# ktonal/mimikit

Measured on AMD Instinct MI355X. Metric: audio samples/sec generated (WaveNet 256-ch mu-law, 16kHz), higher is better.
Workload: dtype f32; 1 GPU; wavenet_cfg4: WaveNet blocks=(10, 10, 10) x 256 ch, 1 cond input(s), mu-law-256, 16 kHz; clips_per_gpu=32, global_clips=32, prompt_samples=3072, decode=greedy, parallelism=clip-shard x1

## Files before the change

### mimikit_amd/csrc/gemm.hip

```cpp
#include "mmk_common.h"
#include "plan_util.h"

namespace mmk {

typedef float f32x4 __attribute__((ext_vector_type(4)));
typedef const __attribute__((address_space(1))) f32x4* gf32x4_ptr;

constexpr int kGemmThreads = 512;
constexpr int kGemmBM = 64, kGemmBN = 128;

__global__ __launch_bounds__(kGemmThreads) void gemm_f32_kernel(const float* __restrict__ A, int64_t lda, int64_t a_batch,
                                                                const float* __restrict__ Wp, float* __restrict__ C,
                                                                int64_t ldc, int64_t c_batch, int M, int n_tiles, int N,
                                                                int K, int k_chunks) {
  extern __shared__ __attribute__((aligned(16))) char smem_raw[];
  float* as = reinterpret_cast<float*>(smem_raw);
  const int ldk = k_chunks * 16 + 4;
  const int tid = threadIdx.x, lane = tid & 63;
  const int wave = __builtin_amdgcn_readfirstlane(tid >> 6);
  const int m_first = blockIdx.y * kGemmBM;
  const int tile = blockIdx.x * (kGemmBN / 16) + wave;
  A += (int64_t)blockIdx.z * a_batch;
  C += (int64_t)blockIdx.z * c_batch;
  const int k4 = k_chunks * 4;
// ... 47 lines not shown
      for (int i = 0; i < 4; ++i) if (col0 + c + i < N) dst[i] = v[i];
  }
}

int launch_gemm_f32(const float* A, int64_t lda, int64_t a_batch, const float* Wp, int n_tiles, int k_chunks, int N, int K,
                    float* C, int64_t ldc, int64_t c_batch, int M, int batch, hipStream_t stream) {
  if (M <= 0 || batch <= 0 || n_tiles <= 0) return MMK_OK;
  size_t lds = (size_t)kGemmBM * (k_chunks * 16 + 4) * sizeof(float);
  const size_t lds_out = (size_t)kGemmBM * (kGemmBN + 4) * sizeof(float);
  if (lds < lds_out) lds = lds_out;
  if (lds > 160 * 1024) return fail(MMK_ERR_UNSUPPORTED, "gemm: K=%d does not fit the LDS stage", K);
  if ((lda % 4) != 0 || (reinterpret_cast<uintptr_t>(A) & 15) != 0) return fail(MMK_ERR_UNSUPPORTED, "gemm: A must be 16-byte aligned with lda %% 4 == 0");
  dim3 grid((n_tiles + kGemmBN / 16 - 1) / (kGemmBN / 16), (M + kGemmBM - 1) / kGemmBM, batch), block(kGemmThreads);
  hipLaunchKernelGGL(gemm_f32_kernel, grid, block, lds, stream, A, lda, a_batch, Wp, C, ldc, c_batch, M, n_tiles, N, K, k_chunks);
  MMK_HIP(hipGetLastError());
  return MMK_OK;
}

constexpr int kTgThreads = 256;
constexpr int kTgBM = 64, kTgBN = 64;
constexpr int kTgCh = 4;
constexpr int kTgLd = kTgCh * 16 + 4;

template <bool WLDS>
__global__ __launch_bounds__(kTgThreads, 2) void gemm_bias_act_kernel(const float* __restrict__ A, int64_t lda, const float* __restrict__ Wp,
                                                                 const float* __restrict__ bias, float* __restrict__ C, int64_t ldc,
                                                                 int M, int n_tiles, int N, int K, int k_chunks, int act, GemmRowMap rm,
                                                                 int k_split, float* __restrict__ partial) {
  extern __shared__ __attribute__((aligned(16))) char smem_raw[];
  float* as = reinterpret_cast<float*>(smem_raw);

  const int tid = threadIdx.x, lane = tid & 63;
  const int wave = __builtin_amdgcn_readfirstlane(tid >> 6);
  const int wm = wave >> 1, wn = wave & 1;
  const int m_first = blockIdx.y * kTgBM;
  const int tile0 = blockIdx.x * (kTgBN / 16) + wn * 2;
  const int a_row = 16 * wave + (lane >> 4) + 4 * ((lane >> 2) & 3), a_col = (lane & 3) * 4;
  const int r0 = m_first + a_row;
  const float* a0 = A + (int64_t)(r0 < M ? r0 : M - 1) * lda + a_col;
  f32x4 va[kTgCh];
  auto load_a = [&](int stage) {
#pragma unroll
    for (int cc = 0; cc < kTgCh; ++cc) {
      const int c = stage * kTgCh + cc;
      const int k = c * 16 + a_col;
      if (k + 3 < K) {
        va[cc] = *reinterpret_cast<const f32x4*>(a0 + c * 16);
      } else {
        for (int i = 0; i < 4; ++i) va[cc][i] = k + i < K ? a0[c * 16 + i] : 0.f;
      }
    }
  };
  auto store_a = [&](int buf) {
    float* dst = as + buf * (kTgBM * kTgLd);
#pragma unroll
    for (int cc = 0; cc < kTgCh; ++cc) {
      *reinterpret_cast<f32x4*>(dst + a_row * kTgLd + cc * 16 + a_col) = va[cc];
    }
  };
  const int t0 = tile0 < n_tiles ? tile0 : n_tiles - 1, t1 = tile0 + 1 < n_tiles ? tile0 + 1 : n_tiles - 1;
  gf32x4_ptr w0 = (gf32x4_ptr)(uintptr_t)Wp + (int64_t)t0 * k_chunks * 64 + lane;
  gf32x4_ptr w1 = (gf32x4_ptr)(uintptr_t)Wp + (int64_t)t1 * k_chunks * 64 + lane;
  f32x4 wc[WLDS ? 1 : kTgCh][2], wx[WLDS ? 1 : kTgCh][2];
  auto load_w = [&](int stage, f32x4 (&w)[WLDS ? 1 : kTgCh][2]) {
    if constexpr (!WLDS) {
#pragma unroll
      for (int cc = 0; cc < kTgCh; ++cc) {
        const int c = stage * kTgCh + cc;
        const int cl = c < k_chunks ? c : k_chunks - 1;
        w[cc][0] = w0[(int64_t)cl * 64];
        w[cc][1] = w1[(int64_t)cl * 64];
      }
    }
  };
  f32x4* ws = reinterpret_cast<f32x4*>(as + 2 * kTgBM * kTgLd);
  const int tl = wn * 2 + wm;
  const int tg = blockIdx.x * (kTgBN / 16) + tl;
// ... 114 lines not shown
  if (rm.group > 0 && i >= rm.kept) return;
  float* dst = rm.group > 0 ? C + (int64_t)g * rm.group_stride + (int64_t)i * rm.row_stride : C + (int64_t)m * ldc;
  for (int col = threadIdx.x; col < N; col += blockDim.x) {
    float v = partial[(int64_t)m * np + col];
    for (int z = 1; z < k_split; ++z) v += partial[((int64_t)z * M + m) * np + col];
    dst[col] = apply_act(v + (bias ? bias[col] : 0.f), act);
  }
}

bool gemm_bias_act_supported(const float* A, int64_t lda, int M, int K) {
  static const int min_m = [] { const char* e = diag_only("MMK_GEMM_MIN_M"); return e ? atoi(e) : 128; }();
  return M >= min_m && K >= 16 && (lda % 4) == 0 && (reinterpret_cast<uintptr_t>(A) & 15) == 0;
}

int gemm_bias_act_k_split(int M, int n_tiles, int k_chunks, int forced = 0) {
  const int wgs = ((n_tiles + kTgBN / 16 - 1) / (kTgBN / 16)) * ((M + kTgBM - 1) / kTgBM);
  const int stages = (k_chunks + kTgCh - 1) / kTgCh;
  int ks = 1;
  while (ks * 2 <= stages && wgs * ks * 2 <= 512 && ks < 8) ks *= 2;
  if (forced > 0) ks = forced < stages ? forced : stages;
  return ks;
}

int64_t gemm_bias_act_partial_floats(int M, int n_tiles, int k_chunks) {
  const int ks = gemm_bias_act_k_split(M, n_tiles, k_chunks);
  return ks > 1 ? (int64_t)ks * M * n_tiles * 16 : 0;
}

int launch_gemm_bias_act(const float* A, int64_t lda, const float* Wp, const float* bias, int n_tiles, int k_chunks, int N, int K, float* C,
                         int64_t ldc, int M, int act, hipStream_t stream, GemmRowMap rm, float* partial, int64_t partial_floats, int forced_k_split) {
  if (M <= 0 || n_tiles <= 0) return MMK_OK;
  if (!gemm_bias_act_supported(A, lda, M, K)) return fail(MMK_ERR_UNSUPPORTED, "gemm_bias_act: needs M >= 128 and a 16-byte aligned A");
  int ks = partial ? gemm_bias_act_k_split(M, n_tiles, k_chunks, forced_k_split) : 1;
  if (ks > 1 && (int64_t)ks * M * n_tiles * 16 > partial_floats) ks = 1;
  dim3 grid((n_tiles + kTgBN / 16 - 1) / (kTgBN / 16), (M + kTgBM - 1) / kTgBM, ks), block(kTgThreads);
  const size_t lds = (size_t)2 * kTgBM * kTgLd * sizeof(float);
  const char* we = diag_only("MMK_GEMM_WLDS");
  if (!(we && we[0] == '0'))
    hipLaunchKernelGGL(gemm_bias_act_kernel<true>, grid, block, lds + (size_t)2 * 4 * kTgCh * 64 * 16, stream, A, lda, Wp, bias, C, ldc, M, n_tiles, N, K,
                       k_chunks, act, rm, ks, partial);
  else
    hipLaunchKernelGGL(gemm_bias_act_kernel<false>, grid, block, lds, stream, A, lda, Wp, bias, C, ldc, M, n_tiles, N, K, k_chunks, act, rm, ks, partial);
  MMK_HIP(hipGetLastError());
  if (ks > 1) {
    hipLaunchKernelGGL(gemm_split_reduce_kernel, dim3(M), dim3(256), 0, stream, partial, ks, M, n_tiles * 16, N, bias, C, ldc, act, rm);
    MMK_HIP(hipGetLastError());
  }
  return MMK_OK;
}

}

extern "C" int mmk_gemm_f32(const float* a, int64_t lda, int64_t a_batch, const float* packed_w, int32_t n_rows, int32_t k_cols, float* c,
                            int64_t ldc, int64_t c_batch, int32_t m_rows, int32_t batch, mmk_stream_t stream) {
  using namespace mmk;
  if (!a || !packed_w || !c || m_rows <= 0 || n_rows <= 0 || k_cols <= 0 || batch <= 0 || lda < k_cols || ldc < n_rows || a_batch < 0 ||
      c_batch < 0)
    return fail(MMK_ERR_INVALID, "gemm: bad arguments");
  if (batch > 1 && (a_batch % 4) != 0) return fail(MMK_ERR_UNSUPPORTED, "gemm: a_batch %% 4 != 0");
  return launch_gemm_f32(a, lda, a_batch, packed_w, (n_rows + 15) / 16, (k_cols + 15) / 16, n_rows, k_cols, c, ldc, c_batch, m_rows, batch,
                         (hipStream_t)stream);
}

extern "C" int64_t mmk_gemm_partial_floats(int32_t m_rows, int32_t n_rows, int32_t k_cols, int32_t k_split) {
  if (m_rows <= 0 || n_rows <= 0 || k_cols <= 0 || k_split < 0) return 0;
// ... 29 lines not shown
```

### mimikit_amd/csrc/mmk_common.h

```cpp
#pragma once
#include <hip/hip_runtime.h>
#include <stdint.h>
#include <stdio.h>
#include <string>
#include <vector>

#include "../../include/mmk.h"

namespace mmk {

void set_error(const char* fmt, ...);
int fail(int code, const char* fmt, ...);

#define MMK_HIP(call)                                                                         \
  do {                                                                                        \
    hipError_t e__ = (call);                                                                  \
    if (e__ != hipSuccess)                                                                    \
      return ::mmk::fail(MMK_ERR_HIP, "%s failed: %s (%s:%d)", #call, hipGetErrorString(e__), \
                         __FILE__, __LINE__);                                                 \
  } while (0)

#define MMK_TRY(expr)            \
  do {                           \
    int rc__ = (expr);           \
// ... 171 lines not shown
};
int launch_sample(const SampleArgs& a, hipStream_t stream);

int launch_stft1024(const float* x, int64_t x_row_stride, int batch, int64_t n_samples, int hop, int center, int reflect, int out_mode,
                    float* out, float* tprev, float momentum, hipStream_t stream);
int launch_stft2048(const float* x, int64_t x_row_stride, int batch, int64_t n_samples, int hop, int center, int reflect, int out_mode,
                    float* out, hipStream_t stream);
int launch_istft2048(const float* spec, const float* mag, int mode, int batch, int64_t n_frames, int hop, float* out, hipStream_t stream);
int launch_gla2048_iter(const float* wave_in, const float* mag, const float* tprev_in, float* tprev_out, float momentum, int batch,
                        int64_t n_frames, int hop, float* wave_out, hipStream_t stream);
int launch_stft_generic(const float* x, int64_t x_row_stride, int batch, int64_t n_samples, int n_fft, int hop, int center, int reflect,
                        int out_mode, float* out, float* tprev, float momentum, hipStream_t stream);
int launch_gemm_f32(const float* A, int64_t lda, int64_t a_batch, const float* Wp, int n_tiles, int k_chunks, int N, int K,
                    float* C, int64_t ldc, int64_t c_batch, int M, int batch, hipStream_t stream);
bool gemm_bias_act_supported(const float* A, int64_t lda, int M, int K);
struct GemmRowMap {
  int32_t group = 0, kept = 0;
  int64_t group_stride = 0, row_stride = 0;
};
int64_t gemm_bias_act_partial_floats(int M, int n_tiles, int k_chunks);
int launch_gemm_bias_act(const float* A, int64_t lda, const float* Wp, const float* bias, int n_tiles, int k_chunks, int N, int K, float* C,
                         int64_t ldc, int M, int act, hipStream_t stream, GemmRowMap rm = GemmRowMap(), float* partial = nullptr,
                         int64_t partial_floats = 0, int forced_k_split = 0);

bool skinny_linear_supported(const float* A, int64_t lda, int M, int K, int k_chunks);
int launch_skinny_linear(const float* A, int64_t lda, const float* Wp, const float* bias, int n_tiles, int k_chunks, int N, int K, float* C,
                         int64_t ldc, int M, int act, hipStream_t stream);

int launch_gru_cell(const float* gi, const float* gh, float* h, int M, int H, hipStream_t stream);
int launch_lstm_cell(const float* gates, int64_t gates_ld, const float* gadd, int64_t gadd_ld, float* h, int64_t h_ld,
                     float* c, int64_t c_ld, float* y, int64_t y_ld, int M, int H, hipStream_t stream);
int launch_rnn_tanh_cell(const float* g, float* h, int M, int H, hipStream_t stream);

}
```

### mimikit_amd/csrc/wavenet_plan.hip

```cpp
#include <stdlib.h>

#include "plan_util.h"
#include "wavenet_chain.h"
#include "wavenet_lpipe.h"
#include "wavenet_persist.h"
#include "wavenet_prefill.h"
#include "wavenet_spipe.h"
#include "wavenet_bpipe.h"

using namespace mmk;

constexpr int kBpipeMinClips = 105;
constexpr int kBpipeAlwaysClips = kSpMaxClips + 1;
static bool bpipe_by_default(int B) { return B >= kBpipeAlwaysClips || (B >= kBpipeMinClips && B % 2 != 0); }

struct WnCall {
  int M = 0;
  const void* in0 = nullptr;
  int64_t in0_rs = 0;
  const float* cond[MMK_MAX_COND] = {nullptr, nullptr, nullptr, nullptr};
  int64_t cond_rs[MMK_MAX_COND] = {0, 0, 0, 0};
  const float* temperature = nullptr;
  const float* uniforms = nullptr;
  int64_t uni_ld = 0;
// ... 23 lines not shown
  std::vector<float*> hist;
  std::vector<float*> cbuf;
  float* ybuf = nullptr;
  float* skipbuf = nullptr;
  float* hid[2] = {nullptr, nullptr};
  int64_t* tau = nullptr;

  hipStream_t cap_stream = nullptr;
  GraphCache gc;

  bool persistent = false;
  int Gc = 0, Gn = 0, Mg = 0, C1 = 0, n_logits_pad = 0;
  static constexpr int kCondBlock = 1024;
  std::vector<int64_t> ring_offset;
  std::vector<int> ring_mask;
  int64_t ring_floats_per_wg = 0;
  PackedLinear cond_all;
  WnLayerTab* layer_tab = nullptr;
  unsigned long long *gran_h = nullptr, *gran_y = nullptr, *gran_skip = nullptr, *gran_hid = nullptr,
                     *gran_logit = nullptr, *gran_idx = nullptr;
  int64_t gran_words = 0;
  float* h_rings = nullptr;
  float* cproj = nullptr;
  float* cpad = nullptr;
  int64_t cpad_rows = 0;
  float* condall = nullptr;
  float* zero_pad = nullptr;
  int64_t pf_P = 0;
  float *pf_h[2] = {nullptr, nullptr}, *pf_y = nullptr, *pf_c = nullptr;
  int32_t* err_flag = nullptr;
  unsigned* xcd_count = nullptr;
  bool xcd_local = false;
  bool chain = false;
  bool lpipe = false;
  unsigned long long *lp_xg = nullptr, *lp_cg = nullptr;
  int64_t lp_gran_words = 0;
  std::vector<PackedLinear> Ac;
  WnChainIter* iter_tab = nullptr;
  float* compose_scratch = nullptr;
  bool spipe = false;
  int last_pair = 0;
  bool bpipe = false;
  float *bp_img = nullptr, *bp_cst = nullptr;
  unsigned* bp_msg = nullptr;
  float *sp_img_chain = nullptr, *sp_img_helper = nullptr, *sp_cst_chain = nullptr, *sp_cst_helper = nullptr, *sp_head_w0 = nullptr, *sp_head_b0 = nullptr;
  unsigned *sp_msg = nullptr, *sp_hidmsg = nullptr, *sp_hidgrp = nullptr;
  WnSpRaw* sp_raw = nullptr;
  const float *sp_fc2_w = nullptr, *sp_fc2_b = nullptr;
// ... 39 lines not shown
      sp_head_b0 = c.take<float>(kSpH1);
      sp_f0p = c.take<float>((int64_t)kSpH1 * C);
      sp_fb0p = c.take<float>(kSpH1);
      sp_fc2p = c.take<float>((int64_t)(kSpQ + 1) * kSpH1);
      sp_fc2bp = c.take<float>(kSpLogitsLd);
      sp_logits = c.take<float>((int64_t)Bmax * kSpLogitsLd);
      if (n_cond == 2) {
        sp_w1cat = c.take<float>((int64_t)L * 2 * C * C1);
        sp_b1cat = c.take<float>((int64_t)L * 2 * C);
      }
      if (bpipe) {
        bp_img = c.take<float>(wn_bpipe_img_floats(L));
        bp_cst = c.take<float>(wn_bpipe_cst_floats(L));
        bp_msg = c.take<unsigned>(wn_bpipe_msg_words(L, Bmax));
      } else {
        sp_msg = c.take<unsigned>(wn_spipe_msg_words(L, C, Bmax) + wn_spipe_hidmsg_words(L, Bmax) + wn_spipe_hidgrp_words(Bmax));
        sp_hidmsg = sp_msg + (sp_msg ? wn_spipe_msg_words(L, C, Bmax) : 0);
        sp_hidgrp = sp_hidmsg + (sp_msg ? wn_spipe_hidmsg_words(L, Bmax) : 0);
      }
      sp_raw = c.take<WnSpRaw>(L);
    }
    h_rings = spipe ? nullptr : c.take<float>((int64_t)Gc * Gn * ring_floats_per_wg);
    cproj = C1 > 0 ? c.take<float>((int64_t)Bmax * kCondBlock * C1) : nullptr;
    if (C1 > 0) {
      int kmax = 16;
      for (int j = 0; j < n_cond; ++j) kmax = (int)round_up(cfg.cond_in_dim[j], 16) > kmax ? (int)round_up(cfg.cond_in_dim[j], 16) : kmax;
      const int64_t prompt_rows = round_up(rf, 32);
      cpad_rows = (int64_t)Bmax * (prompt_rows > kCondBlock ? prompt_rows : kCondBlock);
      cpad = c.take<float>(cpad_rows * kmax);
    }
    condall = (C1 > 0 && !spipe) ? c.take<float>((int64_t)Bmax * kCondBlock * L * 2 * C) : nullptr;
    if (C1 > 0 && !spipe) cond_all.carve(c, false);
    if (chain) {
      for (auto& pl : Ac) pl.carve(c, true);
      iter_tab = c.take<WnChainIter>(L + 1);
      compose_scratch = c.take<float>((int64_t)2 * C * C + 2 * C);
    }
    zero_pad = c.take<float>(64);
    pf_P = round_up(rf, 32);
    pf_h[0] = c.take<float>((int64_t)Bmax * pf_P * C);
    pf_h[1] = c.take<float>((int64_t)Bmax * pf_P * C);
    pf_y = c.take<float>((int64_t)Bmax * pf_P * C);
    pf_c = C1 > 0 ? c.take<float>((int64_t)Bmax * pf_P * C1) : nullptr;
  }

  void layout(Carver& c) {
    const bool bias = cfg.bias != 0;
    if (cfg.q_levels == 0) in0_lin.carve(c, true);
    for (auto& p : cond_lin) p.carve(c, true);
    for (auto& p : A) p.carve(c, bias);
    for (auto& p : Aff) p.carve(c, bias);
    affbuf = Aff.empty() ? nullptr : c.take<float>((int64_t)Bmax * 3 * C);
    for (auto& p : Bm)
// ... 687 lines not shown
      s.uniform_ld = call.uni_ld; s.uni_off = call.uni_off;
      if (k == 0) { s.out = (int64_t*)call.in0; s.out_row_stride = call.in0_rs; }
      else { s.out = reinterpret_cast<int64_t*>(const_cast<float*>(call.cond[k - 1])); s.out_row_stride = call.cond_rs[k - 1]; }
      s.out_tau_off = 1;
      s.tau_ptr = p->tau; s.tau_off = tau_off;
      MMK_TRY(launch_sample(s, st));
    }
  } else {
    LinearArgs a = {};
    p->out_lin.fill(a);
    a.seg[0].x = addr_static(x);
    a.seg[0].ld = p->head_in;
    a.M = M; a.tau_ptr = p->tau; a.tau_off = tau_off;
    a.epilogue = EPI_STORE; a.act = c.head_kind == 1 ? ACT_ABS : ACT_NONE;
    a.out = addr_time(call.in0, c.in_dim, 1, 1, 0);
    a.out_ld = call.in0_rs;
    MMK_TRY(launch_linear(a, st));
  }
  return MMK_OK;
}

static constexpr int kGraphSteps = 8;

__global__ void cond_compact_kernel(const float* __restrict__ src, int64_t clip_stride, int64_t t0, int K, int Kp, int n, int B, float* __restrict__ dst) {
  const int64_t e = (int64_t)blockIdx.x * blockDim.x + threadIdx.x;
  if (e >= (int64_t)B * n * Kp) return;
  const int k = (int)(e % Kp);
  const int64_t row = e / Kp;
  const int b = (int)(row / n), i = (int)(row - (int64_t)b * n);
  dst[e] = k < K ? src[(int64_t)b * clip_stride + (t0 + i) * K + k] : 0.f;
}

static int project_cond(mmk_wavenet_plan* p, const WnCall& call, int j, int col, int64_t t0, int64_t n, float* out, int64_t out_clip_stride, hipStream_t st) {
  const mmk_wavenet_config& c = p->cfg;
  const int K = c.cond_in_dim[j], Kp = (int)round_up(K, 16), B = call.M;
  const char* genv = p->tune.get("MMK_WN_COND_GEMM");
  const int64_t M = (int64_t)B * n;
  if (!(genv && genv[0] == '0') && p->cpad && M <= p->cpad_rows && M < ((int64_t)1 << 31) && gemm_bias_act_supported(p->cpad, Kp, (int)M, K)) {
    const int64_t total = M * Kp;
    hipLaunchKernelGGL(cond_compact_kernel, dim3((unsigned)((total + 255) / 256)), dim3(256), 0, st, call.cond[j], call.cond_rs[j], t0, K, Kp, (int)n, B, p->cpad);
    MMK_HIP(hipGetLastError());
    GemmRowMap rm;
    rm.group = (int)n; rm.kept = (int)n; rm.group_stride = out_clip_stride * p->C1; rm.row_stride = p->C1;
    return launch_gemm_bias_act(p->cpad, Kp, p->cond_lin[j].Wp, p->cond_lin[j].bias, p->cond_lin[j].n_tiles, p->cond_lin[j].k_chunks, c.cond_dim[j], K,
                                out + col, p->C1, (int)M, ACT_NONE, st, rm);
  }
  LinearArgs a = {};
  p->cond_lin[j].fill(a);
  a.seg[0].x = addr_static(call.cond[j] + t0 * K);
  a.seg[0].ld = K;
  a.M = (int)M; a.tau_ptr = nullptr; a.tau_off = 0;
  a.epilogue = EPI_STORE; a.act = ACT_NONE;
  a.out = addr_static(out + col);
  a.out_ld = p->C1;
  a.row_group = (int)n; a.x_group_stride = call.cond_rs[j]; a.out_group_stride = out_clip_stride * p->C1;
  return launch_linear(a, st);
}

static int run_persistent(mmk_wavenet_plan* p, const WnCall& call, int64_t tau0, int64_t n, bool with_head, hipStream_t st) {
  const mmk_wavenet_config& c = p->cfg;
  const MlpHead& h0 = p->heads[0];
  for (int64_t done = 0; done < n;) {
    const int64_t block = (p->lpipe && p->C1 == 0) ? ((int64_t)1 << 20) : (int64_t)p->kCondBlock;
    const int64_t nb = (n - done) < block ? (n - done) : block;
    const int64_t tau_b = tau0 + done;
    if (p->C1 > 0) {
      g_prof_tag = 2;
      for (int j = 0, col = 0; j < p->n_cond; col += c.cond_dim[j], ++j)
// ... 131 lines not shown
    a.h_rings = p->h_rings; a.err_flag = p->err_flag;
    {
      const char* senv = diag_only("MMK_WN_STAMPS");
      a.stamps = (senv && senv[0] == '1') ? reinterpret_cast<unsigned long long*>(p->tau + 8) : nullptr;
    }
    MMK_TRY(launch_wavenet_persist(a, st));
    done += nb;
  }
  return MMK_OK;
}

static int prefill(mmk_wavenet_plan* p, const WnCall& call, int64_t t_begin, int64_t t_end, hipStream_t st) {
  const mmk_wavenet_config& c = p->cfg;
  const int C = p->C, L = p->L, C1 = p->C1, B = call.M;
  const int64_t n = t_end - t_begin, P = p->pf_P;
  MMK_TRY(launch_wn_prefill_embed((const int64_t*)call.in0, call.in0_rs, t_begin, p->emb, c.q_levels, C, (int)n, p->pf_h[0],
                                  P * C, B, st));
  if (C1 > 0) {
    for (int j = 0, col = 0; j < p->n_cond; col += c.cond_dim[j], ++j)
      MMK_TRY(project_cond(p, call, j, col, t_begin, n, p->pf_c, P, st));
  }
  std::vector<int64_t> sfx(L, 0);
  for (int l = L - 2; l >= 0; --l) sfx[l] = sfx[l + 1] + p->dil[l + 1];
  int cur = 0;
  for (int l = 0; l < L; ++l) {
    const int d = p->dil[l];
    const int64_t t_lo = t_end - d > t_begin ? t_end - d : t_begin;
    if (p->lpipe || p->spipe)
      MMK_TRY(launch_wn_lpipe_scatter(p->pf_h[cur], P * C, t_begin, t_lo, (int)(t_end - t_lo), C, B, p->Bmax, p->hist[l], p->ring[l], st));
    else
      MMK_TRY(launch_wn_prefill_scatter(p->pf_h[cur], P * C, t_begin, t_lo, (int)(t_end - t_lo), C, B, p->Mg, p->Gc, p->Gn, p->h_rings,
                                        p->ring_floats_per_wg, p->ring_offset[l], p->ring_mask[l], st));
    if (l == L - 1) break;
    int64_t r_lo = t_end - sfx[l];
    if (r_lo < t_begin + d) r_lo = t_begin + d;
    if (r_lo >= t_end) break;
    const int64_t p0 = r_lo - t_begin;
    const int M = (int)(t_end - r_lo);
    const float* h = p->pf_h[cur];
    {
      WnPrefillArgs a = {};
      a.M = M; a.N = 2 * C; a.n_tiles = p->A[l].n_tiles; a.k_chunks = p->A[l].k_chunks;
      a.nseg = C1 > 0 ? 3 : 2;
      a.seg_k[0] = C; a.seg[0] = h + (p0 - d) * C; a.seg_ld[0] = C; a.seg_batch[0] = P * C;
      a.seg_k[1] = C; a.seg[1] = h + p0 * C; a.seg_ld[1] = C; a.seg_batch[1] = P * C;
      if (C1 > 0) { a.seg_k[2] = C1; a.seg[2] = p->pf_c + p0 * C1; a.seg_ld[2] = C1; a.seg_batch[2] = P * C1; }
      a.wp = p->A[l].Wp; a.bias = p->A[l].bias;
      a.out = p->pf_y + p0 * C; a.out_ld = C; a.out_batch = P * C;
      MMK_TRY(launch_wn_prefill(a, 0, B, st));
    }
    {
      WnPrefillArgs a = {};
      a.M = M; a.N = C; a.n_tiles = C / 16; a.k_chunks = p->Bm[l].k_chunks;
      a.nseg = 1;
      a.seg_k[0] = C; a.seg[0] = p->pf_y + p0 * C; a.seg_ld[0] = C; a.seg_batch[0] = P * C;
      a.wp = p->Bm[l].Wp; a.bias = p->Bm[l].bias;
      a.res_in = h + p0 * C; a.res_ld = C; a.res_batch = P * C;
      a.out = p->pf_h[cur ^ 1] + p0 * C; a.out_ld = C; a.out_batch = P * C;
      MMK_TRY(launch_wn_prefill(a, 1, B, st));
    }
    cur ^= 1;
  }
  return MMK_OK;
}

static int run_steps(mmk_wavenet_plan* p, const WnCall& call, int64_t tau0, int64_t n, bool with_head, hipStream_t st) {
  if (n <= 0) return MMK_OK;
  if (p->persistent) return run_persistent(p, call, tau0, n, with_head, st);
  MMK_TRY(launch_set_i64(p->tau, tau0, st));
  int64_t done = 0;
  if (n >= 2 * kGraphSteps) {
    std::vector<int64_t> key = {call.M, (int64_t)(uintptr_t)call.in0, call.in0_rs, with_head ? 1 : 0,
                                (int64_t)(uintptr_t)call.temperature, (int64_t)(uintptr_t)call.uniforms, call.uni_ld,
                                call.uni_off};
    for (int j = 0; j < p->n_cond; ++j) {
      key.push_back((int64_t)(uintptr_t)call.cond[j]);
      key.push_back(call.cond_rs[j]);
    }
    if (!p->gc.exec || p->gc.key != key) {
      MMK_HIP(hipStreamSynchronize(st));
      p->gc.reset();
      MMK_HIP(hipStreamBeginCapture(p->cap_stream, hipStreamCaptureModeThreadLocal));
// ... 261 lines not shown
```

### mimikit_amd/csrc/wavenet_prefill.h

```cpp
#pragma once
#include "mmk_common.h"

namespace mmk {

struct WnPrefillArgs {
  int32_t M, N, n_tiles, k_chunks;
  int32_t nseg;
  int32_t seg_k[3];
  const float* seg[3]; int64_t seg_ld[3]; int64_t seg_batch[3];
  const float* wp; const float* bias;
  float* out; int64_t out_ld, out_batch;
  const float* res_in; int64_t res_ld, res_batch;
};

int launch_wn_prefill(const WnPrefillArgs& a, int epilogue, int batch, hipStream_t stream);
int launch_wn_prefill_embed(const int64_t* idx, int64_t idx_rs, int64_t t_begin, const float* emb, int q_levels, int C, int n_pos,
                            float* out, int64_t out_batch, int batch, hipStream_t stream);
int launch_wn_prefill_scatter(const float* h, int64_t h_batch, int64_t t_begin, int64_t t_lo, int n_pos, int C, int B, int Mg, int Gc,
                              int Gn, float* rings, int64_t ring_floats_per_wg, int64_t ring_offset, int ring_mask,
                              hipStream_t stream);

}
```

### mimikit_amd/csrc/wavenet_prefill.hip

```cpp
#include "wavenet_prefill.h"
#include "wave_ops.h"

namespace mmk {

typedef float f32x4 __attribute__((ext_vector_type(4)));
typedef const __attribute__((address_space(1))) f32x4* gf32x4_ptr;

constexpr int kPfThreads = 512;
constexpr int kPfBM = 64, kPfBN = 128;

template <int EPI>
__global__ __launch_bounds__(kPfThreads) void wn_prefill_kernel(const WnPrefillArgs a) {
  extern __shared__ __attribute__((aligned(16))) char smem_raw[];
  float* as = reinterpret_cast<float*>(smem_raw);
  int kmax = 16;
  for (int s = 0; s < a.nseg; ++s) kmax = a.seg_k[s] > kmax ? a.seg_k[s] : kmax;
  const int ldk = kmax + 4;
  const int tid = threadIdx.x, lane = tid & 63;
  const int wave = __builtin_amdgcn_readfirstlane(tid >> 6);
  const int m_first = blockIdx.y * kPfBM;
  const int tile = blockIdx.x * (kPfBN / 16) + wave;
  const int b = blockIdx.z;
  const bool live = tile < a.n_tiles;
  gf32x4_ptr w = (gf32x4_ptr)(uintptr_t)a.wp + (int64_t)(live ? tile : 0) * a.k_chunks * 64 + lane;
// ... 47 lines not shown
      } else {
        if (m < a.M && col < a.N) {
          const int64_t o = (int64_t)b * a.out_batch + (int64_t)m * a.out_ld + col;
          a.out[o] = a.res_in[(int64_t)b * a.res_batch + (int64_t)m * a.res_ld + col] + v;
        }
      }
    }
  }
}

int launch_wn_prefill(const WnPrefillArgs& a, int epilogue, int batch, hipStream_t stream) {
  if (a.M <= 0 || batch <= 0 || a.n_tiles <= 0) return MMK_OK;
  int kmax = 16;
  for (int s = 0; s < a.nseg; ++s) kmax = a.seg_k[s] > kmax ? a.seg_k[s] : kmax;
  const size_t lds = (size_t)kPfBM * (kmax + 4) * sizeof(float);
  if (lds > 160 * 1024) return fail(MMK_ERR_UNSUPPORTED, "wavenet prefill: K does not fit the LDS stage");
  dim3 grid((a.n_tiles + kPfBN / 16 - 1) / (kPfBN / 16), (a.M + kPfBM - 1) / kPfBM, batch), block(kPfThreads);
  if (epilogue == 0) hipLaunchKernelGGL((wn_prefill_kernel<0>), grid, block, lds, stream, a);
  else hipLaunchKernelGGL((wn_prefill_kernel<1>), grid, block, lds, stream, a);
  MMK_HIP(hipGetLastError());
  return MMK_OK;
}

__global__ void wn_prefill_embed_kernel(const int64_t* __restrict__ idx, int64_t idx_rs, int64_t t_begin, const float* __restrict__ emb,
                                        int q_levels, int C, int n_pos, float* __restrict__ out, int64_t out_batch) {
  const int b = blockIdx.y;
  const int c4 = C / 4;
  for (int64_t e = blockIdx.x * (int64_t)blockDim.x + threadIdx.x; e < (int64_t)n_pos * c4; e += (int64_t)gridDim.x * blockDim.x) {
    const int p = (int)(e / c4), c = (int)(e - (int64_t)p * c4) * 4;
    const int64_t cls = idx[(int64_t)b * idx_rs + t_begin + p];
    const float nanv = __builtin_nanf("");
    f32x4 v = f32x4{nanv, nanv, nanv, nanv};
    if (cls >= 0 && cls < q_levels) v = *reinterpret_cast<const f32x4*>(emb + cls * C + c);
    *reinterpret_cast<f32x4*>(out + (int64_t)b * out_batch + (int64_t)p * C + c) = v;
  }
}
int launch_wn_prefill_embed(const int64_t* idx, int64_t idx_rs, int64_t t_begin, const float* emb, int q_levels, int C, int n_pos,
                            float* out, int64_t out_batch, int batch, hipStream_t stream) {
  if (n_pos <= 0 || batch <= 0) return MMK_OK;
  const int64_t total = (int64_t)n_pos * (C / 4);
  dim3 grid((unsigned)((total + 255) / 256 > 2048 ? 2048 : (total + 255) / 256), batch);
  hipLaunchKernelGGL(wn_prefill_embed_kernel, grid, dim3(256), 0, stream, idx, idx_rs, t_begin, emb, q_levels, C, n_pos, out, out_batch);
  MMK_HIP(hipGetLastError());
  return MMK_OK;
}

// ... 33 lines not shown
```

Baseline: 829,500 audio samples/s.

## Fuse WaveNet prefill layer GEMMs and read cond rows in place

Adds a fused prefill layer kernel that, per row block, computes the dilated conv GEMM, applies the tanh-sigmoid gate into LDS, then runs the residual GEMM and adds the residual, all in one launch. The intermediate pf_y round trip to global memory and the second launch per layer go away. It also lets the cond projection GEMM read rows directly from the strided cond input instead of compacting them into a padded buffer first. The cost is LDS-heavy kernels with row-block sizes chosen by CU count, and a scalar per-lane A load path in the row-source variant.

```diff
diff --git a/mimikit_amd/csrc/gemm.hip b/mimikit_amd/csrc/gemm.hip
--- a/mimikit_amd/csrc/gemm.hip
+++ b/mimikit_amd/csrc/gemm.hip
@@ -93,11 +93,11 @@
 constexpr int kTgCh = 4;
 constexpr int kTgLd = kTgCh * 16 + 4;
 
-template <bool WLDS>
+template <bool WLDS, bool ROWSRC = false>
 __global__ __launch_bounds__(kTgThreads, 2) void gemm_bias_act_kernel(const float* __restrict__ A, int64_t lda, const float* __restrict__ Wp,
                                                                  const float* __restrict__ bias, float* __restrict__ C, int64_t ldc,
                                                                  int M, int n_tiles, int N, int K, int k_chunks, int act, GemmRowMap rm,
-                                                                 int k_split, float* __restrict__ partial) {
+                                                                 int k_split, float* __restrict__ partial, GemmRowSrc src) {
   extern __shared__ __attribute__((aligned(16))) char smem_raw[];
   float* as = reinterpret_cast<float*>(smem_raw);
 
@@ -110,7 +110,26 @@
   const int r0 = m_first + a_row;
   const float* a0 = A + (int64_t)(r0 < M ? r0 : M - 1) * lda + a_col;
   f32x4 va[kTgCh];
+  const float* arow[ROWSRC ? 4 : 1][4];
+  if constexpr (ROWSRC) {
+#pragma unroll
+    for (int q = 0; q < 4; ++q)
+#pragma unroll
+      for (int j = 0; j < 4; ++j) {
+        const int r = m_first + 16 * wave + 4 * q + j, m = r < M ? r : M - 1;
+        const int g = m / src.group;
+        arow[q][j] = A + (int64_t)g * src.group_stride + (int64_t)(m - g * src.group) * lda + lane;
+      }
+  }
   auto load_a = [&](int stage) {
+    if constexpr (ROWSRC) {
+      const int k = stage * (kTgCh * 16) + lane;
+#pragma unroll
+      for (int q = 0; q < 4; ++q)
+#pragma unroll
+        for (int j = 0; j < 4; ++j) va[q][j] = k < K ? arow[q][j][stage * (kTgCh * 16)] : 0.f;
+      return;
+    }
 #pragma unroll
     for (int cc = 0; cc < kTgCh; ++cc) {
       const int c = stage * kTgCh + cc;
@@ -124,6 +143,13 @@
   };
   auto store_a = [&](int buf) {
     float* dst = as + buf * (kTgBM * kTgLd);
+    if constexpr (ROWSRC) {
+#pragma unroll
+      for (int q = 0; q < 4; ++q)
+#pragma unroll
+        for (int j = 0; j < 4; ++j) dst[(16 * wave + 4 * q + j) * kTgLd + lane] = va[q][j];
+      return;
+    }
 #pragma unroll
     for (int cc = 0; cc < kTgCh; ++cc) {
       *reinterpret_cast<f32x4*>(dst + a_row * kTgLd + cc * 16 + a_col) = va[cc];
@@ -284,6 +310,24 @@
   return ks;
 }
 
+bool gemm_bias_act_rows_supported(int64_t M, int K) { return M < ((int64_t)1 << 31) && gemm_bias_act_supported(nullptr, 0, (int)M, K); }
+
+int launch_gemm_bias_act_rows(const float* A, int64_t lda, GemmRowSrc src, const float* Wp, const float* bias, int n_tiles, int k_chunks, int N, int K,
+                              float* C, int64_t ldc, int M, int act, hipStream_t stream, GemmRowMap rm) {
+  if (M <= 0 || n_tiles <= 0) return MMK_OK;
+  if (!gemm_bias_act_rows_supported(M, K) || src.group <= 0 || lda < K) return fail(MMK_ERR_UNSUPPORTED, "gemm_bias_act (rows in place): needs M >= 128, K >= 16 and a row group");
+  dim3 grid((n_tiles + kTgBN / 16 - 1) / (kTgBN / 16), (M + kTgBM - 1) / kTgBM, 1), block(kTgThreads);
+  const size_t lds = (size_t)2 * kTgBM * kTgLd * sizeof(float);
+  const char* we = diag_only("MMK_GEMM_WLDS");
+  if (!(we && we[0] == '0'))
+    hipLaunchKernelGGL((gemm_bias_act_kernel<true, true>), grid, block, lds + (size_t)2 * 4 * kTgCh * 64 * 16, stream, A, lda, Wp, bias, C, ldc, M, n_tiles, N, K,
+                       k_chunks, act, rm, 1, nullptr, src);
+  else
+    hipLaunchKernelGGL((gemm_bias_act_kernel<false, true>), grid, block, lds, stream, A, lda, Wp, bias, C, ldc, M, n_tiles, N, K, k_chunks, act, rm, 1, nullptr, src);
+  MMK_HIP(hipGetLastError());
+  return MMK_OK;
+}
+
 int64_t gemm_bias_act_partial_floats(int M, int n_tiles, int k_chunks) {
   const int ks = gemm_bias_act_k_split(M, n_tiles, k_chunks);
   return ks > 1 ? (int64_t)ks * M * n_tiles * 16 : 0;
@@ -300,9 +344,9 @@
   const char* we = diag_only("MMK_GEMM_WLDS");
   if (!(we && we[0] == '0'))
     hipLaunchKernelGGL(gemm_bias_act_kernel<true>, grid, block, lds + (size_t)2 * 4 * kTgCh * 64 * 16, stream, A, lda, Wp, bias, C, ldc, M, n_tiles, N, K,
-                       k_chunks, act, rm, ks, partial);
+                       k_chunks, act, rm, ks, partial, GemmRowSrc());
   else
-    hipLaunchKernelGGL(gemm_bias_act_kernel<false>, grid, block, lds, stream, A, lda, Wp, bias, C, ldc, M, n_tiles, N, K, k_chunks, act, rm, ks, partial);
+    hipLaunchKernelGGL(gemm_bias_act_kernel<false>, grid, block, lds, stream, A, lda, Wp, bias, C, ldc, M, n_tiles, N, K, k_chunks, act, rm, ks, partial, GemmRowSrc());
   MMK_HIP(hipGetLastError());
   if (ks > 1) {
     hipLaunchKernelGGL(gemm_split_reduce_kernel, dim3(M), dim3(256), 0, stream, partial, ks, M, n_tiles * 16, N, bias, C, ldc, act, rm);
diff --git a/mimikit_amd/csrc/mmk_common.h b/mimikit_amd/csrc/mmk_common.h
--- a/mimikit_amd/csrc/mmk_common.h
+++ b/mimikit_amd/csrc/mmk_common.h
@@ -217,6 +217,13 @@
 int launch_gemm_bias_act(const float* A, int64_t lda, const float* Wp, const float* bias, int n_tiles, int k_chunks, int N, int K, float* C,
                          int64_t ldc, int M, int act, hipStream_t stream, GemmRowMap rm = GemmRowMap(), float* partial = nullptr,
                          int64_t partial_floats = 0, int forced_k_split = 0);
+struct GemmRowSrc {
+  int32_t group = 0;
+  int64_t group_stride = 0;
+};
+bool gemm_bias_act_rows_supported(int64_t M, int K);
+int launch_gemm_bias_act_rows(const float* A, int64_t lda, GemmRowSrc src, const float* Wp, const float* bias, int n_tiles, int k_chunks, int N, int K,
+                              float* C, int64_t ldc, int M, int act, hipStream_t stream, GemmRowMap rm = GemmRowMap());
 
 bool skinny_linear_supported(const float* A, int64_t lda, int M, int K, int k_chunks);
 int launch_skinny_linear(const float* A, int64_t lda, const float* Wp, const float* bias, int n_tiles, int k_chunks, int N, int K, float* C,
diff --git a/mimikit_amd/csrc/wavenet_plan.hip b/mimikit_amd/csrc/wavenet_plan.hip
--- a/mimikit_amd/csrc/wavenet_plan.hip
+++ b/mimikit_amd/csrc/wavenet_plan.hip
@@ -69,8 +69,6 @@
   int64_t gran_words = 0;
   float* h_rings = nullptr;
   float* cproj = nullptr;
-  float* cpad = nullptr;
-  int64_t cpad_rows = 0;
   float* condall = nullptr;
   float* zero_pad = nullptr;
   int64_t pf_P = 0;
@@ -156,13 +154,6 @@
     }
     h_rings = spipe ? nullptr : c.take<float>((int64_t)Gc * Gn * ring_floats_per_wg);
     cproj = C1 > 0 ? c.take<float>((int64_t)Bmax * kCondBlock * C1) : nullptr;
-    if (C1 > 0) {
-      int kmax = 16;
-      for (int j = 0; j < n_cond; ++j) kmax = (int)round_up(cfg.cond_in_dim[j], 16) > kmax ? (int)round_up(cfg.cond_in_dim[j], 16) : kmax;
-      const int64_t prompt_rows = round_up(rf, 32);
-      cpad_rows = (int64_t)Bmax * (prompt_rows > kCondBlock ? prompt_rows : kCondBlock);
-      cpad = c.take<float>(cpad_rows * kmax);
-    }
     condall = (C1 > 0 && !spipe) ? c.take<float>((int64_t)Bmax * kCondBlock * L * 2 * C) : nullptr;
     if (C1 > 0 && !spipe) cond_all.carve(c, false);
     if (chain) {
@@ -896,28 +887,18 @@
 
 static constexpr int kGraphSteps = 8;
 
-__global__ void cond_compact_kernel(const float* __restrict__ src, int64_t clip_stride, int64_t t0, int K, int Kp, int n, int B, float* __restrict__ dst) {
-  const int64_t e = (int64_t)blockIdx.x * blockDim.x + threadIdx.x;
-  if (e >= (int64_t)B * n * Kp) return;
-  const int k = (int)(e % Kp);
-  const int64_t row = e / Kp;
-  const int b = (int)(row / n), i = (int)(row - (int64_t)b * n);
-  dst[e] = k < K ? src[(int64_t)b * clip_stride + (t0 + i) * K + k] : 0.f;
-}
-
 static int project_cond(mmk_wavenet_plan* p, const WnCall& call, int j, int col, int64_t t0, int64_t n, float* out, int64_t out_clip_stride, hipStream_t st) {
   const mmk_wavenet_config& c = p->cfg;
-  const int K = c.cond_in_dim[j], Kp = (int)round_up(K, 16), B = call.M;
+  const int K = c.cond_in_dim[j], B = call.M;
   const char* genv = p->tune.get("MMK_WN_COND_GEMM");
   const int64_t M = (int64_t)B * n;
-  if (!(genv && genv[0] == '0') && p->cpad && M <= p->cpad_rows && M < ((int64_t)1 << 31) && gemm_bias_act_supported(p->cpad, Kp, (int)M, K)) {
-    const int64_t total = M * Kp;
-    hipLaunchKernelGGL(cond_compact_kernel, dim3((unsigned)((total + 255) / 256)), dim3(256), 0, st, call.cond[j], call.cond_rs[j], t0, K, Kp, (int)n, B, p->cpad);
-    MMK_HIP(hipGetLastError());
+  if (!(genv && genv[0] == '0') && gemm_bias_act_rows_supported(M, K)) {
+    GemmRowSrc rs;
+    rs.group = (int)n; rs.group_stride = call.cond_rs[j];
     GemmRowMap rm;
     rm.group = (int)n; rm.kept = (int)n; rm.group_stride = out_clip_stride * p->C1; rm.row_stride = p->C1;
-    return launch_gemm_bias_act(p->cpad, Kp, p->cond_lin[j].Wp, p->cond_lin[j].bias, p->cond_lin[j].n_tiles, p->cond_lin[j].k_chunks, c.cond_dim[j], K,
-                                out + col, p->C1, (int)M, ACT_NONE, st, rm);
+    return launch_gemm_bias_act_rows(call.cond[j] + t0 * K, K, rs, p->cond_lin[j].Wp, p->cond_lin[j].bias, p->cond_lin[j].n_tiles, p->cond_lin[j].k_chunks,
+                                     c.cond_dim[j], K, out + col, p->C1, (int)M, ACT_NONE, st, rm);
   }
   LinearArgs a = {};
   p->cond_lin[j].fill(a);
@@ -1095,6 +1076,11 @@
   }
   std::vector<int64_t> sfx(L, 0);
   for (int l = L - 2; l >= 0; --l) sfx[l] = sfx[l + 1] + p->dil[l + 1];
+  const char* fenv = p->tune.get("MMK_WN_PREFILL_FUSED");
+  const bool fused = !(fenv && fenv[0] == '0');
+  const char* renv = p->tune.get("MMK_WN_PREFILL_ROWS");
+  const int rows = renv ? atoi(renv) : 0;
+  if (rows < 0 || rows > 128) return fail(MMK_ERR_INVALID, "wavenet: MMK_WN_PREFILL_ROWS=%d outside [0, 128]", rows);
   int cur = 0;
   for (int l = 0; l < L; ++l) {
     const int d = p->dil[l];
@@ -1111,26 +1097,37 @@
     const int64_t p0 = r_lo - t_begin;
     const int M = (int)(t_end - r_lo);
     const float* h = p->pf_h[cur];
-    {
-      WnPrefillArgs a = {};
-      a.M = M; a.N = 2 * C; a.n_tiles = p->A[l].n_tiles; a.k_chunks = p->A[l].k_chunks;
-      a.nseg = C1 > 0 ? 3 : 2;
-      a.seg_k[0] = C; a.seg[0] = h + (p0 - d) * C; a.seg_ld[0] = C; a.seg_batch[0] = P * C;
-      a.seg_k[1] = C; a.seg[1] = h + p0 * C; a.seg_ld[1] = C; a.seg_batch[1] = P * C;
-      if (C1 > 0) { a.seg_k[2] = C1; a.seg[2] = p->pf_c + p0 * C1; a.seg_ld[2] = C1; a.seg_batch[2] = P * C1; }
-      a.wp = p->A[l].Wp; a.bias = p->A[l].bias;
-      a.out = p->pf_y + p0 * C; a.out_ld = C; a.out_batch = P * C;
-      MMK_TRY(launch_wn_prefill(a, 0, B, st));
-    }
-    {
-      WnPrefillArgs a = {};
-      a.M = M; a.N = C; a.n_tiles = C / 16; a.k_chunks = p->Bm[l].k_chunks;
-      a.nseg = 1;
-      a.seg_k[0] = C; a.seg[0] = p->pf_y + p0 * C; a.seg_ld[0] = C; a.seg_batch[0] = P * C;
-      a.wp = p->Bm[l].Wp; a.bias = p->Bm[l].bias;
-      a.res_in = h + p0 * C; a.res_ld = C; a.res_batch = P * C;
-      a.out = p->pf_h[cur ^ 1] + p0 * C; a.out_ld = C; a.out_batch = P * C;
-      MMK_TRY(launch_wn_prefill(a, 1, B, st));
+    if (fused && wn_prefill_layer_supported(C, C1, p->ksz[l], p->A[l].n_tiles, p->A[l].k_chunks, p->has_res[l] ? p->Bm[l].n_tiles : 0, p->Bm[l].k_chunks)) {
+      WnPrefillLayerArgs a = {};
+      a.M = M; a.C1 = C1; a.rows = rows; a.d = d;
+      a.h = h + p0 * C; a.h_batch = P * C;
+      if (C1 > 0) { a.c = p->pf_c + p0 * C1; a.c_batch = P * C1; }
+      a.wa = p->A[l].Wp; a.bias_a = p->A[l].bias; a.ka_chunks = p->A[l].k_chunks;
+      a.wb = p->Bm[l].Wp; a.bias_b = p->Bm[l].bias; a.kb_chunks = p->Bm[l].k_chunks;
+      a.out = p->pf_h[cur ^ 1] + p0 * C; a.out_batch = P * C;
+      MMK_TRY(launch_wn_prefill_layer(a, B, st));
+    } else {
+      {
+        WnPrefillArgs a = {};
+        a.M = M; a.N = 2 * C; a.n_tiles = p->A[l].n_tiles; a.k_chunks = p->A[l].k_chunks;
+        a.nseg = C1 > 0 ? 3 : 2;
+        a.seg_k[0] = C; a.seg[0] = h + (p0 - d) * C; a.seg_ld[0] = C; a.seg_batch[0] = P * C;
+        a.seg_k[1] = C; a.seg[1] = h + p0 * C; a.seg_ld[1] = C; a.seg_batch[1] = P * C;
+        if (C1 > 0) { a.seg_k[2] = C1; a.seg[2] = p->pf_c + p0 * C1; a.seg_ld[2] = C1; a.seg_batch[2] = P * C1; }
+        a.wp = p->A[l].Wp; a.bias = p->A[l].bias;
+        a.out = p->pf_y + p0 * C; a.out_ld = C; a.out_batch = P * C;
+        MMK_TRY(launch_wn_prefill(a, 0, B, st));
+      }
+      {
+        WnPrefillArgs a = {};
+        a.M = M; a.N = C; a.n_tiles = C / 16; a.k_chunks = p->Bm[l].k_chunks;
+        a.nseg = 1;
+        a.seg_k[0] = C; a.seg[0] = p->pf_y + p0 * C; a.seg_ld[0] = C; a.seg_batch[0] = P * C;
+        a.wp = p->Bm[l].Wp; a.bias = p->Bm[l].bias;
+        a.res_in = h + p0 * C; a.res_ld = C; a.res_batch = P * C;
+        a.out = p->pf_h[cur ^ 1] + p0 * C; a.out_ld = C; a.out_batch = P * C;
+        MMK_TRY(launch_wn_prefill(a, 1, B, st));
+      }
     }
     cur ^= 1;
   }
diff --git a/mimikit_amd/csrc/wavenet_prefill.h b/mimikit_amd/csrc/wavenet_prefill.h
--- a/mimikit_amd/csrc/wavenet_prefill.h
+++ b/mimikit_amd/csrc/wavenet_prefill.h
@@ -14,6 +14,19 @@
 };
 
 int launch_wn_prefill(const WnPrefillArgs& a, int epilogue, int batch, hipStream_t stream);
+
+struct WnPrefillLayerArgs {
+  int32_t M, C1;
+  int32_t rows;
+  const float* h; int64_t h_batch;
+  int32_t d;
+  const float* c; int64_t c_batch;
+  const float* wa; const float* bias_a; int32_t ka_chunks;
+  const float* wb; const float* bias_b; int32_t kb_chunks;
+  float* out; int64_t out_batch;
+};
+bool wn_prefill_layer_supported(int C, int C1, int ksz, int a_tiles, int a_chunks, int b_tiles, int b_chunks);
+int launch_wn_prefill_layer(const WnPrefillLayerArgs& a, int batch, hipStream_t stream);
 int launch_wn_prefill_embed(const int64_t* idx, int64_t idx_rs, int64_t t_begin, const float* emb, int q_levels, int C, int n_pos,
                             float* out, int64_t out_batch, int batch, hipStream_t stream);
 int launch_wn_prefill_scatter(const float* h, int64_t h_batch, int64_t t_begin, int64_t t_lo, int n_pos, int C, int B, int Mg, int Gc,
diff --git a/mimikit_amd/csrc/wavenet_prefill.hip b/mimikit_amd/csrc/wavenet_prefill.hip
--- a/mimikit_amd/csrc/wavenet_prefill.hip
+++ b/mimikit_amd/csrc/wavenet_prefill.hip
@@ -93,6 +93,208 @@
   return MMK_OK;
 }
 
+constexpr int kPlThreads = 512, kPlC = 256, kPlLd = kPlC + 4;
+
+template <int RT>
+__global__ __launch_bounds__(kPlThreads) void wn_prefill_layer_kernel(const WnPrefillLayerArgs a) {
+  extern __shared__ __attribute__((aligned(16))) char smem_raw[];
+  float* as = reinterpret_cast<float*>(smem_raw);
+  constexpr int BM = RT * 16, PF = RT;
+  const int tid = threadIdx.x, lane = tid & 63;
+  const int wave = __builtin_amdgcn_readfirstlane(tid >> 6);
+  const int m_first = blockIdx.x * BM;
+  const int b = blockIdx.y;
+  const float* hb = a.h + (int64_t)b * a.h_batch;
+  const float* x = as + (lane & 15) * kPlLd + 4 * (lane >> 4);
+  const int n = lane & 15;
+  const int nseg = a.C1 > 0 ? 3 : 2;
+  f32x4 pre[PF];
+  auto fetch = [&](int s, int half) {
+    const int K = s < 2 ? kPlC : a.C1, k4 = K / 4;
+    const float* base = s == 0 ? hb - (int64_t)a.d * kPlC : s == 1 ? hb : a.c + (int64_t)b * a.c_batch;
+#pragma unroll
+    for (int j = 0; j < PF; ++j) {
+      const int q = tid + (half * PF + j) * kPlThreads, m = q / k4, c = (q - m * k4) * 4;
+      f32x4 v = f32x4{0.f, 0.f, 0.f, 0.f};
+      if (m < BM && m_first + m < a.M) v = *reinterpret_cast<const f32x4*>(base + (int64_t)(m_first + m) * K + c);
+      pre[j] = v;
+    }
+  };
+  auto put = [&](int s, int half) {
+    const int k4 = (s < 2 ? kPlC : a.C1) / 4;
+#pragma unroll
+    for (int j = 0; j < PF; ++j) {
+      const int q = tid + (half * PF + j) * kPlThreads, m = q / k4, c = (q - m * k4) * 4;
+      if (m < BM) *reinterpret_cast<f32x4*>(as + m * kPlLd + c) = pre[j];
+    }
+  };
+  f32x4 acc[RT][4];
+#pragma unroll
+  for (int rt = 0; rt < RT; ++rt)
+#pragma unroll
+    for (int ct = 0; ct < 4; ++ct) acc[rt][ct] = f32x4{0.f, 0.f, 0.f, 0.f};
+  auto chunk = [&](const f32x4 (&wf)[4], int c) {
+    f32x4 xr[2];
+    xr[0] = *reinterpret_cast<const f32x4*>(x + c * 16);
+#pragma unroll
+    for (int rt = 0; rt < RT; ++rt) {
+      if (rt + 1 < RT) xr[(rt + 1) & 1] = *reinterpret_cast<const f32x4*>(x + (rt + 1) * 16 * kPlLd + c * 16);
+#pragma unroll
+      for (int i = 0; i < 4; ++i) {
+#pragma unroll
+        for (int ct = 0; ct < 4; ++ct) acc[rt][ct] = __builtin_amdgcn_mfma_f32_16x16x4f32(xr[rt & 1][i], wf[ct][i], acc[rt][ct], 0, 0, 0);
+      }
+    }
+    __builtin_amdgcn_sched_group_barrier(0x100, 2, 0);
+#pragma unroll
+    for (int rt = 0; rt < RT; ++rt) {
+      __builtin_amdgcn_sched_group_barrier(0x008, 16, 0);
+      if (rt + 2 < RT) __builtin_amdgcn_sched_group_barrier(0x100, 1, 0);
+    }
+  };
+  fetch(0, 0);
+  put(0, 0);
+  fetch(0, 1);
+  put(0, 1);
+  __syncthreads();
+  {
+    const int64_t wts = (int64_t)a.ka_chunks * 64;
+    gf32x4_ptr w = (gf32x4_ptr)(uintptr_t)a.wa + (int64_t)(wave * 4) * wts + lane;
+    int c0 = 0;
+    for (int s = 0; s < nseg; ++s) {
+      if (s + 1 < nseg) fetch(s + 1, 0);
+      const int kc = (s < 2 ? kPlC : a.C1) / 16;
+      f32x4 wa[4], wb[4];
+#pragma unroll
+      for (int ct = 0; ct < 4; ++ct) wa[ct] = w[ct * wts + (int64_t)c0 * 64];
+      int c = 0;
+      for (; c + 1 < kc; c += 2) {
+#pragma unroll
+        for (int ct = 0; ct < 4; ++ct) wb[ct] = w[ct * wts + (int64_t)(c0 + c + 1) * 64];
+        __builtin_amdgcn_sched_group_barrier(0x020, 4, 0);
+        chunk(wa, c);
+#pragma unroll
+        for (int ct = 0; ct < 4; ++ct) wa[ct] = w[ct * wts + (int64_t)(c0 + (c + 2 < kc ? c + 2 : kc - 1)) * 64];
+        __builtin_amdgcn_sched_group_barrier(0x020, 4, 0);
+        chunk(wb, c + 1);
+      }
+      if (c < kc) chunk(wa, c);
+      c0 += kc;
+      __syncthreads();
+      if (s + 1 < nseg) {
+        put(s + 1, 0);
+        fetch(s + 1, 1);
+        put(s + 1, 1);
+        __syncthreads();
+      }
+    }
+  }
+  const bool odd = n & 1;
+#pragma unroll
+  for (int ct = 0; ct < 4; ++ct) {
+    const int tile = wave * 4 + ct;
+    const float bias = a.bias_a ? a.bias_a[tile * 16 + n] : 0.f;
+    float* yp = as + (4 * (lane >> 4) + (odd ? 1 : 0)) * kPlLd + tile * 8 + (n >> 1);
+#pragma unroll
+    for (int rt = 0; rt < RT; ++rt) {
+      const float v0 = acc[rt][ct][0] + bias, v1 = acc[rt][ct][1] + bias, v2 = acc[rt][ct][2] + bias, v3 = acc[rt][ct][3] + bias;
+      const float q0 = dpp_xor1(odd ? v0 : v1), q1 = dpp_xor1(odd ? v2 : v3);
+      const float f0 = odd ? q0 : v0, g0 = odd ? v1 : q0, f1 = odd ? q1 : v2, g1 = odd ? v3 : q1;
+      yp[(rt * 16) * kPlLd] = tanhf(f0) * sigmoidf_(g0);
+      yp[(rt * 16 + 2) * kPlLd] = tanhf(f1) * sigmoidf_(g1);
+    }
+  }
+  __syncthreads();
+  f32x4 rc[RT][2];
+#pragma unroll
+  for (int rt = 0; rt < RT; ++rt) rc[rt][0] = rc[rt][1] = f32x4{0.f, 0.f, 0.f, 0.f};
+  {
+    const int64_t wts = (int64_t)a.kb_chunks * 64;
+    gf32x4_ptr w = (gf32x4_ptr)(uintptr_t)a.wb + (int64_t)(wave * 2) * wts + lane;
+    constexpr int kc = kPlC / 16;
+    auto chunk2 = [&](const f32x4 (&wf)[2], int c) {
+      f32x4 xr[2];
+      xr[0] = *reinterpret_cast<const f32x4*>(x + c * 16);
+#pragma unroll
+      for (int rt = 0; rt < RT; ++rt) {
+        if (rt + 1 < RT) xr[(rt + 1) & 1] = *reinterpret_cast<const f32x4*>(x + (rt + 1) * 16 * kPlLd + c * 16);
+#pragma unroll
+        for (int i = 0; i < 4; ++i) {
+          rc[rt][0] = __builtin_amdgcn_mfma_f32_16x16x4f32(xr[rt & 1][i], wf[0][i], rc[rt][0], 0, 0, 0);
+          rc[rt][1] = __builtin_amdgcn_mfma_f32_16x16x4f32(xr[rt & 1][i], wf[1][i], rc[rt][1], 0, 0, 0);
+        }
+      }
+      __builtin_amdgcn_sched_group_barrier(0x100, 2, 0);
+#pragma unroll
+      for (int rt = 0; rt < RT; ++rt) {
+        __builtin_amdgcn_sched_group_barrier(0x008, 8, 0);
+        if (rt + 2 < RT) __builtin_amdgcn_sched_group_barrier(0x100, 1, 0);
+      }
+    };
+    f32x4 wa[2] = {w[0], w[wts]}, wb[2];
+    for (int c = 0; c < kc; c += 2) {
+      wb[0] = w[(int64_t)(c + 1) * 64];
+      wb[1] = w[wts + (int64_t)(c + 1) * 64];
+      __builtin_amdgcn_sched_group_barrier(0x020, 2, 0);
+      chunk2(wa, c);
+      const int cn = c + 2 < kc ? c + 2 : kc - 1;
+      wa[0] = w[(int64_t)cn * 64];
+      wa[1] = w[wts + (int64_t)cn * 64];
+      __builtin_amdgcn_sched_group_barrier(0x020, 2, 0);
+      chunk2(wb, c + 1);
+    }
+  }
+  float* ob = a.out + (int64_t)b * a.out_batch;
+#pragma unroll
+  for (int ct = 0; ct < 2; ++ct) {
+    const int col = (wave * 2 + ct) * 16 + n;
+    const float bias = a.bias_b ? a.bias_b[col] : 0.f;
+#pragma unroll
+    for (int rt = 0; rt < RT; ++rt) {
+#pragma unroll
+      for (int r = 0; r < 4; ++r) {
+        const int m = m_first + rt * 16 + 4 * (lane >> 4) + r;
+        const float v = rc[rt][ct][r] + bias;
+        if (m < a.M) ob[(int64_t)m * kPlC + col] = hb[(int64_t)m * kPlC + col] + v;
+      }
+    }
+  }
+}
+
+bool wn_prefill_layer_supported(int C, int C1, int ksz, int a_tiles, int a_chunks, int b_tiles, int b_chunks) {
+  return C == kPlC && ksz == 2 && C1 >= 0 && C1 <= 256 && C1 % 16 == 0 && a_tiles == 2 * kPlC / 16 && a_chunks == (2 * kPlC + C1) / 16 &&
+         b_tiles >= kPlC / 16 && b_chunks == kPlC / 16;
+}
+
+template <int RT>
+static int launch_wn_prefill_layer_rt(const WnPrefillLayerArgs& a, int batch, hipStream_t stream) {
+  const size_t lds = (size_t)RT * 16 * kPlLd * sizeof(float);
+  MMK_HIP(hipFuncSetAttribute(reinterpret_cast<const void*>(&wn_prefill_layer_kernel<RT>), hipFuncAttributeMaxDynamicSharedMemorySize, (int)lds));
+  hipLaunchKernelGGL((wn_prefill_layer_kernel<RT>), dim3((a.M + RT * 16 - 1) / (RT * 16), batch), dim3(kPlThreads), lds, stream, a);
+  MMK_HIP(hipGetLastError());
+  return MMK_OK;
+}
+
+int launch_wn_prefill_layer(const WnPrefillLayerArgs& a, int batch, hipStream_t stream) {
+  if (a.M <= 0 || batch <= 0) return MMK_OK;
+  static const int n_cu = [] {
+    int dev = 0;
+    hipDeviceProp_t prop;
+    return (hipGetDevice(&dev) == hipSuccess && hipGetDeviceProperties(&prop, dev) == hipSuccess && prop.multiProcessorCount > 0) ? prop.multiProcessorCount : 256;
+  }();
+  const int blocks128 = (a.M + 127) / 128;
+  const int64_t rounds = ((int64_t)batch * blocks128 + n_cu - 1) / n_cu;
+  int64_t blocks = rounds * n_cu / batch;
+  if (blocks < blocks128) blocks = blocks128;
+  const int rows = a.rows > 0 ? a.rows : (int)((a.M + blocks - 1) / blocks);
+  const int rt = (rows + 15) / 16;
+  if (rt <= 4) return launch_wn_prefill_layer_rt<4>(a, batch, stream);
+  if (rt == 5) return launch_wn_prefill_layer_rt<5>(a, batch, stream);
+  if (rt == 6) return launch_wn_prefill_layer_rt<6>(a, batch, stream);
+  if (rt == 7) return launch_wn_prefill_layer_rt<7>(a, batch, stream);
+  return launch_wn_prefill_layer_rt<8>(a, batch, stream);
+}
+
 __global__ void wn_prefill_embed_kernel(const int64_t* __restrict__ idx, int64_t idx_rs, int64_t t_begin, const float* __restrict__ emb,
                                         int q_levels, int C, int n_pos, float* __restrict__ out, int64_t out_batch) {
   const int b = blockIdx.y;
```

New measurement: 836,300 audio samples/s (median of 6 runs). No clear change (+0.8%).
